# Drehrumbum/viterbi.dll

Measured on AMD Instinct MI355X. Metric: decoded Mbit/s per GPU on batched 768-bit DAB FIC frames; bit-exact vs AVX2 ref, higher is better.
Workload: dtype u8

## Files before the change

### __graft_entry__.py

```python
import os
import sys

ROOT = os.path.dirname(os.path.abspath(__file__))
if ROOT not in sys.path:
    sys.path.insert(0, ROOT)

import _vitpkg


def build():
    V = _vitpkg.load_package()
    V.build(force=False)
    V.lib()
    for sym in V.EXPORTS:
        getattr(V.lib(), sym)
    diag = os.path.join(os.path.dirname(V.LIB_PATH_DEFAULT), "libviterbi_diag.so")
    if not os.path.exists(diag) or os.path.getmtime(diag) < os.path.getmtime(V.LIB_PATH_DEFAULT):
        V.build(extra=["-DVIT_DIAG_SPEC"], out=diag)
    O = _vitpkg.load_oracle()
    O.build()
    O.lib()
    if _vitpkg.load_ref().build():
        _vitpkg.load_ref().lib()


def smoke():
    import numpy as np
    import torch

    V = _vitpkg.load_package()
    O = _vitpkg.load_oracle()
    assert torch.cuda.is_available(), "smoke() needs a GPU"
    assert V.device_count() >= 1, "libviterbi found no gfx950 device"
    assert V.initialize()
    framebits, n = 768, 64
    sym = np.concatenate([O.noisy_frames(n // 2, framebits, seed=7),
                          O.uniform_symbols((n // 2) * O.sym_len(framebits), seed=9).reshape(n // 2, -1)])
    want = O.decode_batch(framebits, sym, ge=True)
    d_sym = torch.from_numpy(sym).to("cuda:0")
    d_out = torch.zeros((n, framebits // 8), dtype=torch.uint8, device="cuda:0")
    V.decode_batch_dev(d_sym, d_out, framebits, n)
    torch.cuda.synchronize()
    got = d_out.cpu().numpy()
    assert np.array_equal(got, want), "GPU decode differs from the oracle"
    reps = 65
    d_big = d_sym.repeat(reps, 1)
    d_big_out = torch.zeros((n * reps, framebits // 8), dtype=torch.uint8, device="cuda:0")
    V.decode_batch_dev(d_big, d_big_out, framebits, n * reps)
    torch.cuda.synchronize()
    assert bool((d_big_out.view(reps, n, -1) == d_out.unsqueeze(0)).all()), "packed kernel differs from the oracle"
    rc, one = V.deconvolve(framebits, sym[0].astype(np.uint32))
    assert rc == 0 and np.array_equal(one, want[0])
    rs = 12
    rng = np.random.default_rng(3)
    cols = np.stack([O.rs_encode(rng.integers(0, 256, 110, dtype=np.uint8)) for _ in range(rs)], axis=1)
    p = cols.reshape(-1).copy()
    p[5 * rs + 3] ^= 0x5A
    p[77 * rs + 3] ^= 0x11
    p[9 * rs + 7] ^= 0xC3
    rc_ref, out_ref = O.rs_check_superframe(p, rs)
    rc_gpu, out_gpu = V.RScheckSuperframe(p, 0, rs)
    assert rc_gpu == rc_ref == 3 and np.array_equal(out_gpu, out_ref)
    print("smoke ok: %d + %d frames bit-exact (latency + packed kernel), deconvolve rc=0, RScheckSuperframe=%d"
          % (n, n * reps, rc_gpu))


if __name__ == "__main__":
    {"build": build, "smoke": smoke}[sys.argv[1] if len(sys.argv) > 1 else "build"]()
```

### viterbi.dll_amd/csrc/vit_pk.hip

```cpp
#include <cstdlib>
#include <mutex>

#include "vit_internal.h"
#include "vit_pk_dev.h"

namespace {

constexpr int TAB_BYTES = 2048;
constexpr int DEC_BLOCK = 512;
constexpr unsigned PK_SPLIT_DEN = 8;

#ifndef VIT_TAB_STATIC
#define VIT_TAB_STATIC 1
#endif
struct Lanes {
    u32 toff[5];
};


#ifndef VIT_SWZ_ALL
#define VIT_SWZ_ALL 1
#endif
#ifndef VIT_K3
#define VIT_K3 2
// ... 90 lines not shown
        return;
#endif
#if VIT_PAIR_LSB
        const u32 z = (u32)__builtin_amdgcn_ds_bpermute((int)((lane & 1u) << 2), (int)W(n0));
#else
        const u32 z = (u32)__builtin_amdgcn_ds_swizzle((int)W(n0), 0);
#endif
        exchange<4 - RHO>(A, B, W(n0), W(n1), lane);
#if VIT_K3 == 2
        u32 K;
        {
            const u32 w = z + C.rc;
            asm("v_pk_ashrrev_i16 %0, 15, %1 op_sel_hi:[0,1]\n\t"
                "v_and_or_b32 %0, %0, %2, %3"
                : "=&v"(K)
                : "v"(w), "s"(0x003F003Fu), "v"(C.hi));
        }
#elif VIT_K3
        u32 K;
        asm("v_pk_add_u16 %0, %1, %2\n\t"
            "v_pk_ashrrev_i16 %0, 15, %0 op_sel_hi:[0,1]\n\t"
            "v_and_or_b32 %0, %0, %3, %4"
            : "=&v"(K)
            : "v"(z), "s"(C.rc + 0x00010000u), "s"(0x003F003Fu), "v"(C.hi));
#else
        const u32 w = z + C.rc;
        const u32 t = (w >> 15) & 0x00010001u;
        const u32 K = t * 63u + C.hi;
#endif
        A = W(__builtin_elementwise_sub_sat(U(A), U(K)));
        B = W(__builtin_elementwise_sub_sat(U(B), U(K)));
    } else {
#ifdef VIT_DIAG_SKIP_X
        if constexpr (RHO == 2) {
            A = W(n0);
            B = W(n1);
            return;
        }
#endif
        exchange<4 - RHO>(A, B, W(n0), W(n1), lane);
    }
}

template <int V, int J, int JEND, bool HIST>
struct Steps {
    static DEV void run(u32& A, u32& B, u32& acc0, u32& acc1, const char* tab, const Lanes& L, u32 lane,
                        const Consts& C) {
        constexpr int RHO = (V + J) % 5;
#if VIT_TAB_STATIC
        const u32 mt = *reinterpret_cast<const __attribute__((address_space(3))) u32*>(L.toff[RHO] + (u32)(J * 64));
#else
        const u32 mt = *reinterpret_cast<const u32*>(tab + L.toff[RHO] + J * 64);
#endif
        acs_step<RHO, J, HIST>(A, B, acc0, acc1, mt, lane, C);
        Steps<V, J + 1, JEND, HIST>::run(A, B, acc0, acc1, tab, L, lane, C);
    }
};
template <int V, int JEND, bool HIST>
struct Steps<V, JEND, JEND, HIST> {
    static DEV void run(u32&, u32&, u32&, u32&, const char*, const Lanes&, u32, const Consts&) {}
};
template <bool HIST, int N = 16>
DEV void steps16(u32 v, u32& A, u32& B, u32& acc0, u32& acc1, const char* th, const Lanes& L, u32 lane, const Consts& C) {
    switch (v) {
        case 0: Steps<0, 0, N, HIST>::run(A, B, acc0, acc1, th, L, lane, C); break;
        case 1: Steps<1, 0, N, HIST>::run(A, B, acc0, acc1, th, L, lane, C); break;
        case 2: Steps<2, 0, N, HIST>::run(A, B, acc0, acc1, th, L, lane, C); break;
        case 3: Steps<3, 0, N, HIST>::run(A, B, acc0, acc1, th, L, lane, C); break;
        default: Steps<4, 0, N, HIST>::run(A, B, acc0, acc1, th, L, lane, C); break;
    }
}
DEV void steps6(u32 v, u32& A, u32& B, u32& acc0, u32& acc1, const char* th, const Lanes& L, u32 lane, const Consts& C) {
    steps16<true, 6>(v, A, B, acc0, acc1, th, L, lane, C);
    acc0 >>= 7;
    acc1 >>= 7;
}

typedef u32 v32u __attribute__((ext_vector_type(32)));
constexpr u32 VREG_BLOCKS = 32;

constexpr u32 DUMP_GROUP = 16;
constexpr u32 SEG_BLOCKS = VREG_BLOCKS + DUMP_GROUP + 1u;

__host__ __device__ inline u32 pk_reg_blocks(u32 nb) {
    if (nb <= DUMP_GROUP + 1u) return 0;
    const u32 r = nb - (DUMP_GROUP + 1u);
    return r < VREG_BLOCKS ? r : VREG_BLOCKS;
}
__host__ __device__ inline u32 pk_img_stride(u32 maxfb) { return ((maxfb + 31u) >> 5) + 2u; }
__host__ __device__ inline u32 pk_scratch_words(u32 maxfb) {
    u32 nblk = (maxfb + VIT_TAIL + 15u) >> 4;
    if (nblk > SEG_BLOCKS) nblk = SEG_BLOCKS;
    const u32 tail = (nblk - pk_reg_blocks(nblk)) * 16u;
    const u32 span = tail > 256u ? tail : 256u;
    const u32 bl = 5u * ((span + 79u) / 80u);
    return (bl + 31u) >> 5;
}
struct PkLayout {
    u32 dec_bytes;
    u32 img_off;
    u32 total;
    u32 maxfb;
};
__host__ __device__ inline PkLayout pk_layout(u32 maxfb) {
    const u32 nb = (maxfb + VIT_TAIL + 15u) >> 4;
    PkLayout l;
    l.maxfb = maxfb;
    l.dec_bytes = (nb - pk_reg_blocks(nb) - 1u) * DEC_BLOCK;
    const u32 scratch = 64u * 4u * pk_scratch_words(maxfb), img = 16u * pk_img_stride(maxfb);
    u32 tabregion = DEC_BLOCK + scratch + img;
    tabregion = tabregion > (u32)TAB_BYTES ? ((tabregion + 15u) & ~15u) : (u32)TAB_BYTES;
    l.img_off = l.dec_bytes + DEC_BLOCK + scratch;
    l.total = l.dec_bytes + tabregion;
    return l;
}

constexpr u32 P_ZERO = 252u;
#ifndef VIT_TB_WARM
#define VIT_TB_WARM 30
#endif
#ifndef VIT_TB16
#define VIT_TB16 (VIT_TB_WARM == 30)
#endif
constexpr u32 TB_WARM = VIT_TB_WARM;
#ifndef VIT_TB_WARM_HARD
#define VIT_TB_WARM_HARD 90
#endif
#ifndef VIT_TB_HARD_MISSES
#define VIT_TB_HARD_MISSES 8
#endif
constexpr u32 TB_WARM_HARD = VIT_TB_WARM_HARD, TB_HARD_MISSES = VIT_TB_HARD_MISSES;

#ifdef VIT_DIAG_SPEC
__device__ unsigned long long g_diag_spec[8];
#define SPEC_COUNT(i) do { if (lane == 0) atomicAdd(&g_diag_spec[i], 1ull); } while (0)
#define SPEC_COUNT_N(i, n) do { if (lane == 0) atomicAdd(&g_diag_spec[i], (unsigned long long)(n)); } while (0)
#else
#define SPEC_COUNT(i) do { } while (0)
#endif

DEV u32 dec_slot(u32 lane) { return acs_pair(lane) * 256u + (31u - acs_l5(lane)) * 8u; }

template <int JJ>
DEV void tb_step(u32& PC, u32& kb, u32 x) {
    const u32 w = *reinterpret_cast<const __attribute__((address_space(3))) unsigned short*>((x & ~511u) | PC);
    kb = __builtin_amdgcn_ubfe(w, (x >> 5) & 15u, 1u);
    const u32 t = ((PC >> (JJ - 2)) & 4u) | (kb << JJ);
    PC = bfi((1u << JJ) | 4u, t, PC);
}

template <bool RECORD, int JA>
DEV void tb_loop(u32& PC, u32* scratch, int i_from, int i_to, bool on, u32 i_start, u32 xbase) {
    u32 cur = 0;
    for (int i = i_from; i >= i_to; i -= 5) {
#define TB_ONE(K)                                                                  \
    {                                                                              \
        const int ii = i - (K);                                                    \
        u32 kb = 0;                                                                \
        if (on && (u32)ii <= i_start) tb_step<3 + (JA + (K)) % 5>(PC, kb, xbase + ((u32)ii << 5)); \
        if (RECORD) {                                                              \
            cur |= kb << (ii & 31);                                                \
            if ((ii & 31) == 0) {                                                  \
                if (on) scratch[ii >> 5] = cur;                                    \
                cur = 0;                                                           \
            }                                                                      \
        }                                                                          \
    }
        TB_ONE(0) TB_ONE(1) TB_ONE(2) TB_ONE(3) TB_ONE(4)
#undef TB_ONE
    }
}
template <bool RECORD>
DEV void tb_run(u32& PC, u32* scratch, int i_from, int i_to, bool on, u32 i_start, u32 xbase, u32 j0) {
    switch ((j0 + 1u) % 5u) {
        case 0: tb_loop<RECORD, 0>(PC, scratch, i_from, i_to, on, i_start, xbase); break;
        case 1: tb_loop<RECORD, 1>(PC, scratch, i_from, i_to, on, i_start, xbase); break;
        case 2: tb_loop<RECORD, 2>(PC, scratch, i_from, i_to, on, i_start, xbase); break;
        case 3: tb_loop<RECORD, 3>(PC, scratch, i_from, i_to, on, i_start, xbase); break;
        default: tb_loop<RECORD, 4>(PC, scratch, i_from, i_to, on, i_start, xbase); break;
    }
}

#ifndef VIT_TB_INLINE
#define VIT_TB_INLINE 1
#endif
#if VIT_TB_INLINE
DEV
#else
__device__ __attribute__((noinline))
#endif
u32 traceback_part(const char* dec, u32* scratch, u32* img, u32 fstride, u32 lane, u32 ts, u32 te, u32 te_max,
                       u32 slot0, u32 P_top, u32& warm, u32 dmask = 0xFFFFFFFFu) {
#ifdef VIT_DIAG_NO_TB
    return P_top;
#endif
    const u32 fi = lane >> 4, q = lane & 15u;
    const u32 span = te_max > ts ? te_max - ts : 0u;
    if (span == 0) return P_top;
    const u32 BL = 5u * ((span + 79u) / 80u);
    const u32 tbase = ts + q * BL;
    const bool has_work = tbase < te;
    const u32 i_last = has_work ? te - 1u - tbase : 0u;
    const u32 q_top = te > ts ? (te - 1u - ts) / BL : 0u;
    const u32 i_warm = BL - 1u + warm;
    const u32 i_start = i_last < i_warm ? i_last : i_warm;
    const bool fixed = has_work && i_last <= i_warm;
    const u32 C = (fi >> 1) * 256u + (fi & 1u) * 2u;
    const u32 dbase = (u32)(uintptr_t)(const __attribute__((address_space(3))) char*)dec;
    if (dbase & 511u) __builtin_trap();
    const u32 xbase = ((tbase - slot0 * 16u) << 5) + dbase;
    const u32 j0 = (4u + 5u - ((ts + 5u - 1u) % 5u)) % 5u;
    const u32 PC_top = P_top | C;

    u32 P = fixed ? PC_top : (P_ZERO | C), P_out = PC_top;
    tb_run<false>(P, scratch, (int)i_warm, (int)BL, has_work, i_start, xbase, j0);
    u32 P_in = P;
    tb_run<true>(P, scratch, (int)BL - 1, 0, has_work, i_start, xbase, j0);
    if (has_work) P_out = P;
    for (int pass = 0; pass < 17; pass++) {
        const u32 nxt = __shfl_down(P_out, 1);
        const u32 new_in = (q < q_top) ? nxt : PC_top;
        const bool changed = has_work && !fixed && new_in != P_in;
        const unsigned long long miss = __ballot(changed);
        if (miss == 0) break;
#ifdef VIT_DIAG_SPEC
        if (pass == 0 && warm == TB_WARM && (u32)__popcll(miss) >= TB_HARD_MISSES) SPEC_COUNT(7);
#endif
        if (pass == 0 && warm == TB_WARM && (u32)__popcll(miss) >= TB_HARD_MISSES) warm = TB_WARM_HARD;
        if (changed) P_in = new_in;
        P = new_in;
        tb_run<true>(P, scratch, (int)BL - 1, 0, changed, BL - 1u, xbase, j0);
        if (changed) P_out = P;
    }
    if (has_work) {
        const u32 nvalid = i_last + 1u < BL ? i_last + 1u : BL;
        const u32 nw = (BL + 31u) >> 5;
        for (u32 w = 0; w < nw; w++) {
            const u32 lo = 32u * w;
            const u32 cnt = nvalid > lo ? nvalid - lo : 0u;
            const u32 mask = cnt >= 32u ? 0xFFFFFFFFu : ((1u << cnt) - 1u);
            const u32 val = ~scratch[w] & mask;
            const u32 b0 = tbase - VIT_TAIL + lo;
            const u32 d = b0 >> 5, sft = b0 & 31u;
            if (val) {
                atomicOr(&img[fi * fstride + (d & dmask)], val << sft);
                if (sft) atomicOr(&img[fi * fstride + ((d + 1u) & dmask)], val >> (32u - sft));
            }
        }
    }
    return __shfl(P_out, (int)(fi * 16u)) & 0xFCu;
}

struct Tb16 {
    u32 sh[5], jj[5], mk[5];
};
DEV u32 bfi_v(u32 mask, u32 a, u32 b) {
    u32 d;
    asm("v_bfi_b32 %0, %1, %2, %3" : "=v"(d) : "v"(mask), "v"(a), "v"(b));
    return d;
}
template <int II, bool REC>
DEV void tb16_step(u32& PC, u32& cur, const Tb16& L) {
    constexpr int r = II % 5, blk = (6 + II) >> 4, idx = (6 + II) & 15;
    const u32 w = *reinterpret_cast<const __attribute__((address_space(3))) unsigned short*>(PC + (u32)(blk * DEC_BLOCK));
    u32 kb;
    asm("v_bfe_u32 %0, %1, %2, 1" : "=v"(kb) : "v"(w), "n"(idx));
    const u32 m = (PC >> L.sh[r]) & 4u;
    const u32 t = (kb << L.jj[r]) | m;
    PC = bfi_v(L.mk[r], t, PC);
    if constexpr (REC) cur |= kb << II;
}
template <int IFROM, int ITO, bool REC>
struct Tb16Run {
    static DEV void run(u32& PC, u32& cur, const Tb16& L) {
        tb16_step<IFROM, REC>(PC, cur, L);
        if constexpr (IFROM > ITO) Tb16Run<IFROM - 1, ITO, REC>::run(PC, cur, L);
    }
};
template <bool SPEC = false, bool TOMEM = false>
DEV u32 traceback_part16(const char* dec, u32* img, u32 fstride, u32 lane, u32 lo, u32 nl, u32 slot0, u32 P_top, u32 dmask,
                         uint8_t* gout = nullptr, u32* p_spec = nullptr, u32* misses = nullptr) {
#ifdef VIT_DIAG_NO_TB
    return P_top;
#endif
    constexpr int W = 30;
    const u32 fi = lane >> 4, q = lane & 15u;
    const u32 tbase = lo + q * 16u;
    const bool has_work = q < nl;
    const u32 above = SPEC ? 3u : nl - q;
    const bool fixed = has_work && above <= 2u;
    const u32 C = (fi >> 1) * 256u + (fi & 1u) * 2u;
    const u32 dbase = (u32)(uintptr_t)(const __attribute__((address_space(3))) char*)dec;
    if (dbase & 511u) __builtin_trap();
    const u32 bbq = dbase + ((lo >> 4) - slot0 + q) * DEC_BLOCK;
    Tb16 L;
    {
        const u32 c = (tbase + 4u) % 5u;
#pragma unroll
        for (int r = 0; r < 5; r++) {
            const u32 e = (c + r) % 5u, JJ = 7u - e;
            L.sh[r] = JJ - 2u;
            L.jj[r] = JJ;
            L.mk[r] = (1u << JJ) | 4u;
        }
    }
    const u32 PC_top = P_top | C;
    u32 P = (fixed ? PC_top : (P_ZERO | C)) | bbq, P_out = PC_top, cur = 0;
    if (has_work && above >= 3u) Tb16Run<15 + W, 32, false>::run(P, cur, L);
    if (has_work && above >= 2u) Tb16Run<31, 16, false>::run(P, cur, L);
    u32 P_in = P & 0x1FFu;
    if (has_work) {
        Tb16Run<15, 0, true>::run(P, cur, L);
        P_out = P & 0x1FFu;
    }
    for (int pass = 0; pass < 17; pass++) {
        const u32 nxt = (u32)__builtin_amdgcn_update_dpp(0, (int)P_out, 0x101, 0xF, 0xF, true);
        const u32 new_in = (q + 1u < nl) ? nxt : (SPEC ? P_in : PC_top);
        const bool changed = has_work && !fixed && new_in != P_in;
        if constexpr (SPEC) {
            const unsigned long long miss = __ballot(changed);
            if (pass == 0) *misses = (u32)__popcll(miss);
            if (miss == 0) break;
        } else {
#ifdef VIT_DIAG_SPEC
            {
                const unsigned long long miss = __ballot(changed);
                if (pass == 0) SPEC_COUNT_N(5, __popcll(miss));
                if (miss) SPEC_COUNT(6);
            }
#endif
            if (!__any(changed)) break;
        }
        if (changed) {
            P_in = new_in;
            P = new_in | bbq;
            cur = 0;
            Tb16Run<15, 0, true>::run(P, cur, L);
            P_out = P & 0x1FFu;
        }
    }
    if (has_work) {
        const u32 h = (tbase - VIT_TAIL) >> 4;
        if constexpr (TOMEM) {
            const u32 v = __builtin_bitreverse32(~cur & 0xFFFFu);
            gout[2u * h] = (uint8_t)(v >> 24);
            gout[2u * h + 1u] = (uint8_t)(v >> 16);
        } else {
            reinterpret_cast<unsigned short*>(img + fi * fstride)[((h >> 1) & dmask) * 2u + (h & 1u)] = (unsigned short)~cur;
        }
    }
    if constexpr (SPEC) *p_spec = __shfl(P_in, (int)(fi * 16u + nl - 1u)) & 0xFCu;
    return __shfl(P_out, (int)(fi * 16u)) & 0xFCu;
}

#ifdef VIT_DIAG_TIMES
__device__ unsigned long long g_diag_times[16384 * 4];
#endif
template <bool SYM32, bool ROT>
__global__ __launch_bounds__(64, 4) void vit_pk_kernel(const uint8_t* __restrict__ sym, uint8_t* __restrict__ out,
                                                        const vit_frame_desc* __restrict__ desc, u32 framebits_uniform,
                                                        long long nframes, PkLayout lay, u32 vmax,
                                                        const unsigned* __restrict__ split_gate, u32 renorm_c) {
    if (split_gate && (unsigned long long)*split_gate * PK_SPLIT_DEN >= (unsigned long long)nframes) return;
#ifdef VIT_DIAG_TIMES
    const unsigned long long diag_t0 = __builtin_amdgcn_s_memrealtime();
#endif
    extern __shared__ __attribute__((aligned(16))) char lds[];
    char* dec = lds;
    char* tab = lds + lay.dec_bytes;
    u32* img = reinterpret_cast<u32*>(lds + lay.img_off);
    const u32 lane = threadIdx.x;
    const long long f0 = (long long)blockIdx.x * 4;
    u32 prio_slot = 0;
#if VIT_PRIO
    {
        u32 hwid;
        asm volatile("s_getreg_b32 %0, hwreg(HW_REG_HW_ID)" : "=s"(hwid));
        prio_slot = hwid & 3u;
#ifdef VIT_PRIO_FIRST
// ... 132 lines not shown
    __syncthreads();
#pragma nounroll
    for (u32 i = lane; i < 4u * fstride; i += 64u) img[i] = 0;

#ifdef VIT_DIAG_TIMES
    const unsigned long long diag_t1 = __builtin_amdgcn_s_memrealtime();
#endif
    const u32 fi = lane >> 4;
    const u32 t_fb = fi == 0 ? fbits[0] : fi == 1 ? fbits[1] : fi == 2 ? fbits[2] : fbits[3];
    const u32 t_T = t_fb ? t_fb + VIT_TAIL : 0u;
    u32* scratch = reinterpret_cast<u32*>(tab + DEC_BLOCK) + lane * pk_scratch_words(maxfb);
#if VIT_TB16
    if (fbits[0] == fbits[1] && fbits[1] == fbits[2] && fbits[2] == fbits[3] && (maxfb & 15u) == 0) {
        u32 hi = T_max, slot0 = R, P16 = P_ZERO;
        for (;;) {
            const u32 lo = hi > 256u + VIT_TAIL ? hi - 256u : VIT_TAIL;
            P16 = traceback_part16(dec, img, fstride, lane, lo, (hi - lo) >> 4, slot0, P16, 0xFFFFFFFFu);
            if (lo == VIT_TAIL) break;
            const u32 d = slot0 < DUMP_GROUP ? slot0 : DUMP_GROUP;
            __syncthreads();
            for (u32 sl = DUMP_GROUP; sl >= d; sl--)
                *reinterpret_cast<uint2*>(dec + sl * DEC_BLOCK + dslot) = *reinterpret_cast<const uint2*>(dec + (sl - d) * DEC_BLOCK + dslot);
            const u32 g0 = slot0 - d;
#pragma unroll
            for (u32 b = 0; b < VREG_BLOCKS; b++)
                if (b >= g0 && b < slot0)
                    *reinterpret_cast<uint2*>(dec + (b - g0) * DEC_BLOCK + dslot) = make_uint2(r1[b], r0[b]);
            __syncthreads();
            slot0 = g0;
            hi = lo;
        }
    } else {
#endif
    const u32 t_lo = R * 16u;
    u32 warm = TB_WARM;
    u32 P_part = traceback_part(dec, scratch, img, fstride, lane, t_lo > VIT_TAIL ? t_lo : VIT_TAIL, t_T, T_max, R,
                                P_ZERO, warm);
    for (u32 g1 = R; g1 > 0;) {
        const u32 g0 = g1 > DUMP_GROUP ? g1 - DUMP_GROUP : 0u;
        __syncthreads();
#pragma unroll
        for (u32 b = 0; b < VREG_BLOCKS; b++)
            if (b >= g0 && b < g1)
                *reinterpret_cast<uint2*>(dec + (b - g0) * DEC_BLOCK + dslot) = make_uint2(r1[b], r0[b]);
        __syncthreads();
        const u32 tsg = g0 ? g0 * 16u : VIT_TAIL, tend = g1 * 16u;
        const u32 te = t_T < tend ? t_T : tend, te_max = T_max < tend ? T_max : tend;
        const u32 P_top = t_T > tend ? P_part : P_ZERO;
        P_part = traceback_part(dec, scratch, img, fstride, lane, tsg, te, te_max, g0, P_top, warm);
        g1 = g0;
    }
#if VIT_TB16
    }
#endif
    __syncthreads();

#ifdef VIT_DIAG_TIMES
    if (threadIdx.x == 0 && blockIdx.x < 16384u) {
        u32 hwid;
        asm volatile("s_getreg_b32 %0, hwreg(HW_REG_HW_ID)" : "=s"(hwid));
        g_diag_times[blockIdx.x * 4u + 0u] = diag_t0;
        g_diag_times[blockIdx.x * 4u + 1u] = diag_t1;
        g_diag_times[blockIdx.x * 4u + 2u] = __builtin_amdgcn_s_memrealtime();
        g_diag_times[blockIdx.x * 4u + 3u] = hwid;
    }
#endif
    {
        const u32 k = lane >> 4, j = lane & 15u;
        const u32 fb_k = k == 0 ? fbits[0] : k == 1 ? fbits[1] : k == 2 ? fbits[2] : fbits[3];
        const size_t oo_k = k == 0 ? ooff[0] : k == 1 ? ooff[1] : k == 2 ? ooff[2] : ooff[3];
        const u32 nbytes = (fb_k + 7u) >> 3;
        uint8_t* o = out + oo_k;
        const u32* im = img + k * fstride;
        if ((((u32)oo_k | nbytes) & 3u) == 0) {
#pragma nounroll
            for (u32 m = j; m < (nbytes >> 2); m += 16u)
                reinterpret_cast<u32*>(o)[m] = __builtin_bswap32(__builtin_bitreverse32(im[m]));
        } else {
#pragma nounroll
            for (u32 b = j; b < nbytes; b += 16u) {
                const u32 byte = (im[b >> 2] >> (8u * (b & 3u))) & 0xFFu;
                o[b] = (uint8_t)(__builtin_bitreverse32(byte) >> 24);
            }
        }
    }
}

constexpr u32 LONG_LDS_BLOCKS = DUMP_GROUP + 1u;
constexpr u32 LONG_KEEP = DUMP_GROUP;
constexpr u32 SPEC_BLOCKS = LONG_LDS_BLOCKS + 2u;

constexpr u32 IMG_RING = 16;

__host__ __device__ inline PkLayout pk_layout_long(u32 maxfb) {
    PkLayout l;
    l.maxfb = maxfb;
    l.dec_bytes = DUMP_GROUP * DEC_BLOCK;
    const u32 scratch = 64u * 4u * pk_scratch_words(maxfb), img = 4u * 4u * IMG_RING;
    u32 tabregion = DEC_BLOCK + scratch + img;
    tabregion = tabregion > (u32)TAB_BYTES ? ((tabregion + 15u) & ~15u) : (u32)TAB_BYTES;
    l.img_off = l.dec_bytes + DEC_BLOCK + scratch;
    l.total = l.dec_bytes + tabregion;
    return l;
}
static_assert(SPEC_BLOCKS * DEC_BLOCK <= DUMP_GROUP * DEC_BLOCK + (u32)TAB_BYTES, "an in-flight part must fit dec + the dead table");

struct Carry {
    u32 a0, b0, a1, b1, a2, b2, a3, b3;
};
DEV void carry_put(Carry& c, int d, u32 x, u32 y) {
    asm volatile(
        "s_cmp_lt_i32 %[d], 16\n\t"
        "s_cbranch_scc1 .Lcy_end%=\n\t"
        "s_cmp_lg_u32 %[d], 16\n\t"
        "s_cbranch_scc1 .Lcy_1%=\n\t"
        "v_mov_b32 %[a0], %[x]\n\t"
        "v_mov_b32 %[b0], %[y]\n\t"
        "s_branch .Lcy_end%=\n"
        ".Lcy_1%=:\n\t"
        "s_cmp_lg_u32 %[d], 17\n\t"
        "s_cbranch_scc1 .Lcy_2%=\n\t"
        "v_mov_b32 %[a1], %[x]\n\t"
        "v_mov_b32 %[b1], %[y]\n\t"
        "s_branch .Lcy_end%=\n"
        ".Lcy_2%=:\n\t"
        "s_cmp_lg_u32 %[d], 18\n\t"
        "s_cbranch_scc1 .Lcy_3%=\n\t"
        "v_mov_b32 %[a2], %[x]\n\t"
        "v_mov_b32 %[b2], %[y]\n\t"
        "s_branch .Lcy_end%=\n"
        ".Lcy_3%=:\n\t"
        "v_mov_b32 %[a3], %[x]\n\t"
        "v_mov_b32 %[b3], %[y]\n"
        ".Lcy_end%=:"
        : [a0] "+v"(c.a0), [b0] "+v"(c.b0), [a1] "+v"(c.a1), [b1] "+v"(c.b1), [a2] "+v"(c.a2), [b2] "+v"(c.b2), [a3] "+v"(c.a3), [b3] "+v"(c.b3)
        : [d] "s"(d), [x] "v"(x), [y] "v"(y)
        : "scc");
}
DEV void carry_to_lds(const Carry& c, char* dec, u32 dslot, u32 first, u32 n) {
    if (n > 0u) *reinterpret_cast<uint2*>(dec + (first + 0u) * DEC_BLOCK + dslot) = make_uint2(c.a0, c.b0);
    if (n > 1u) *reinterpret_cast<uint2*>(dec + (first + 1u) * DEC_BLOCK + dslot) = make_uint2(c.a1, c.b1);
    if (n > 2u) *reinterpret_cast<uint2*>(dec + (first + 2u) * DEC_BLOCK + dslot) = make_uint2(c.a2, c.b2);
    if (n > 3u) *reinterpret_cast<uint2*>(dec + (first + 3u) * DEC_BLOCK + dslot) = make_uint2(c.a3, c.b3);
}
DEV u32 pack_rows(u32 P) {
    return (u32)__builtin_amdgcn_readlane((int)P, 0) | ((u32)__builtin_amdgcn_readlane((int)P, 16) << 8) |
           ((u32)__builtin_amdgcn_readlane((int)P, 32) << 16) | ((u32)__builtin_amdgcn_readlane((int)P, 48) << 24);
}

#ifndef VIT_LONG_BASE_PRIO
#define VIT_LONG_BASE_PRIO 1
#endif
#ifndef VIT_LONG_INFLIGHT
#define VIT_LONG_INFLIGHT 1
#endif

DEV void wave_sync() { asm volatile("s_waitcnt lgkmcnt(0)" ::: "memory"); }

template <bool SYM32>
__global__ __launch_bounds__(64, 4) void vit_pk_long_kernel(const uint8_t* __restrict__ sym, uint8_t* __restrict__ out,
                                                             const vit_frame_desc* __restrict__ desc,
                                                             u32 framebits_uniform, long long nframes, PkLayout lay,
                                                             uint2* spill, u32 spill_blocks, unsigned* counter,
                                                             u32 ngroups, u32 short_max,
                                                             const unsigned* __restrict__ split_gate, u32 renorm_c, u32 nsimd) {
    extern __shared__ __attribute__((aligned(16))) char lds[];
// ... 392 lines not shown
#endif
bool vit_pk_supported(uint32_t max_framebits) {
    if (max_framebits < 2 || max_framebits > PK_MAX_FRAMEBITS || (max_framebits % 2u) != 0) return false;
    const u32 nblk = (max_framebits + VIT_TAIL + 15u) >> 4;
    return (nblk <= SEG_BLOCKS ? pk_layout(max_framebits) : pk_layout_long(max_framebits)).total <= 160u * 1024u;
}

struct ScratchCtx {
    void* buf = nullptr;
    size_t cap = 0;
    hipEvent_t ev = nullptr;
    int dev = -1;
    bool bins_clean = false;
    hipStream_t side = nullptr;
    hipEvent_t ev_fork = nullptr, ev_join = nullptr;
    void drop_side() {
        if (side) (void)hipStreamDestroy(side);
        if (ev_fork) (void)hipEventDestroy(ev_fork);
        if (ev_join) (void)hipEventDestroy(ev_join);
        side = nullptr;
        ev_fork = ev_join = nullptr;
    }
    ~ScratchCtx() {
        drop_side();
        if (buf) (void)hipFree(buf);
        if (ev) (void)hipEventDestroy(ev);
    }
};
constexpr int PK_MAX_DEVS = 64;
struct ScratchCtxs {
    ScratchCtx by_dev[PK_MAX_DEVS];
};
thread_local ScratchCtxs t_scratch;
constexpr size_t SCRATCH_HDR = 16384;
constexpr int64_t SORT_MIN_FRAMES = 16;

bool sort_enabled() {
    static const bool on = getenv("VITERBI_AMD_NO_SORT") == nullptr;
    return on;
}

hipError_t vit_launch_pk(const void* d_symbols, bool sym32, uint8_t* d_out, const vit_frame_desc* d_desc,
                         uint32_t framebits, uint32_t max_framebits, int64_t nframes, hipStream_t stream, bool renorm_ge) {
    const u32 rc = pk_renorm_const(renorm_ge);
    const uint8_t* d_sym = static_cast<const uint8_t*>(d_symbols);
    if (sym32 && (reinterpret_cast<uintptr_t>(d_symbols) & 15u)) return hipErrorInvalidValue;
    if (nframes <= 0) return hipSuccess;
    if (!vit_pk_supported(max_framebits)) return hipErrorInvalidValue;
    hipError_t e;
    int dev = 0;
    if ((e = hipGetDevice(&dev)) != hipSuccess) return e;
    {
        static uint64_t optin_done = 0;
        const void* ks[6] = {reinterpret_cast<const void*>(vit_pk_kernel<false, false>),
                             reinterpret_cast<const void*>(vit_pk_kernel<true, false>),
                             reinterpret_cast<const void*>(vit_pk_kernel<false, true>),
                             reinterpret_cast<const void*>(vit_pk_kernel<true, true>),
                             reinterpret_cast<const void*>(vit_pk_long_kernel<false>),
                             reinterpret_cast<const void*>(vit_pk_long_kernel<true>)};
        if ((e = vit_optin_dynamic_lds(ks, 6, 160 * 1024, dev, &optin_done)) != hipSuccess) return e;
    }
    const long long groups = (nframes + 3) / 4;
    if (groups > 0x7FFFFFFFLL) return hipErrorInvalidValue;
    const u32 nblk = (max_framebits + VIT_TAIL + 15u) >> 4;
#ifdef VIT_FORCE_LONG
    const bool is_long = true;
#else
    const bool is_long = nblk > SEG_BLOCKS;
#endif
    const bool sort = d_desc != nullptr && nframes >= SORT_MIN_FRAMES && sort_enabled();
    const PkLayout lay = is_long ? pk_layout_long(max_framebits) : pk_layout(max_framebits);
    long long grid = groups;
    if (is_long) {
        u32 per_cu = (160u * 1024u) / lay.total;
        if (per_cu > 16u) per_cu = 16u;
        grid = (long long)per_cu * vit_device_cus(dev);
        if (grid > groups) grid = groups;
    }
    const bool need_counter = is_long;
    auto launch_short = [&](long long g, const PkLayout& l, u32 vmax, const unsigned* gate, bool may_rotate) {
        u32 per_cu = (160u * 1024u) / l.total;
        if (per_cu > 16u) per_cu = 16u;
        const bool rot = may_rotate && g <= (long long)per_cu * vit_device_cus(dev) && g > 4ll * vit_device_cus(dev);
#define VIT_LAUNCH_SHORT(S32, R)                                                                                          \
    hipLaunchKernelGGL((vit_pk_kernel<S32, R>), dim3((unsigned)g), dim3(64), l.total, stream, d_sym, d_out, d_desc, framebits, \
                       (long long)nframes, l, vmax, gate, rc)
        if (sym32) {
            if (rot) VIT_LAUNCH_SHORT(true, true);
            else VIT_LAUNCH_SHORT(true, false);
        } else {
            if (rot) VIT_LAUNCH_SHORT(false, true);
            else VIT_LAUNCH_SHORT(false, false);
        }
#undef VIT_LAUNCH_SHORT
    };
    if (!need_counter && !sort) {
        launch_short(grid, lay, lay.maxfb, nullptr, true);
        return hipGetLastError();
    }
    const u32 spill_blocks = is_long ? nblk - LONG_KEEP : 0u;
    const size_t desc_bytes = sort ? (((size_t)nframes * sizeof(vit_frame_desc) + 255u) & ~(size_t)255u) : 0u;
    const size_t need = SCRATCH_HDR + desc_bytes + (size_t)grid * spill_blocks * DEC_BLOCK;
    if (dev < 0 || dev >= PK_MAX_DEVS) return hipErrorInvalidDevice;
    ScratchCtx& sc = t_scratch.by_dev[dev];
    if (sc.cap < need) {
        if (sc.buf) (void)hipFree(sc.buf);
        sc.buf = nullptr;
        sc.cap = 0;
        sc.bins_clean = false;
        if (sc.ev) (void)hipEventDestroy(sc.ev);
        sc.ev = nullptr;
        if ((e = hipMalloc(&sc.buf, need + need / 4)) != hipSuccess) return e;
        sc.cap = need + need / 4;
        sc.dev = dev;
        if ((e = hipEventCreateWithFlags(&sc.ev, hipEventDisableTiming)) != hipSuccess) return e;
    } else if ((e = hipStreamWaitEvent(stream, sc.ev, 0)) != hipSuccess) {
        return e;
    }
    char* base = static_cast<char*>(sc.buf);
    if (sort) {
        vit_frame_desc* sorted = reinterpret_cast<vit_frame_desc*>(base + SCRATCH_HDR);
        if ((e = vit_sort_descs_launch(d_desc, sorted, nframes, max_framebits, reinterpret_cast<unsigned*>(base + 256),
                                       stream, &sc.bins_clean, reinterpret_cast<unsigned*>(base))) != hipSuccess)
            return e;
        d_desc = sorted;
    }
    unsigned* counter = reinterpret_cast<unsigned*>(base);
    if (need_counter && !sort && (e = hipMemsetAsync(base, 0, 256, stream)) != hipSuccess) return e;
    if (is_long) {
        const u32 short_max = sort ? PK_SHORT_MAX : 0u;
        const unsigned* gate = sort ? reinterpret_cast<const unsigned*>(base + 256) + VIT_SORT_BINS + ((PK_SHORT_MAX + 7u) >> 3) : nullptr;
        uint2* spill = reinterpret_cast<uint2*>(base + SCRATCH_HDR + desc_bytes);
        hipStream_t ls = stream;
        if (short_max) {
            if (!sc.side) {
                if ((e = hipStreamCreateWithFlags(&sc.side, hipStreamNonBlocking)) != hipSuccess) return e;
                if ((e = hipEventCreateWithFlags(&sc.ev_fork, hipEventDisableTiming)) != hipSuccess) return e;
                if ((e = hipEventCreateWithFlags(&sc.ev_join, hipEventDisableTiming)) != hipSuccess) return e;
            }
            if ((e = hipEventRecord(sc.ev_fork, stream)) != hipSuccess) return e;
            if ((e = hipStreamWaitEvent(sc.side, sc.ev_fork, 0)) != hipSuccess) return e;
            ls = sc.side;
        }
        if (sym32)
            hipLaunchKernelGGL(vit_pk_long_kernel<true>, dim3((unsigned)grid), dim3(64), lay.total, ls, d_sym, d_out,
                               d_desc, framebits, (long long)nframes, lay, spill, spill_blocks, counter, (u32)groups,
                               short_max, gate, rc, 4u * (u32)vit_device_cus(dev));
        else
            hipLaunchKernelGGL(vit_pk_long_kernel<false>, dim3((unsigned)grid), dim3(64), lay.total, ls, d_sym, d_out,
                               d_desc, framebits, (long long)nframes, lay, spill, spill_blocks, counter, (u32)groups,
                               short_max, gate, rc, 4u * (u32)vit_device_cus(dev));
        if (short_max && (e = hipGetLastError()) == hipSuccess) {
            const PkLayout lsh = pk_layout(PK_SHORT_MAX);
            launch_short(groups, lsh, max_framebits, gate, false);
            if ((e = hipGetLastError()) != hipSuccess) return e;
            if ((e = hipEventRecord(sc.ev_join, sc.side)) != hipSuccess) return e;
            if ((e = hipStreamWaitEvent(stream, sc.ev_join, 0)) != hipSuccess) return e;
        }
    } else {
        launch_short(grid, lay, lay.maxfb, nullptr, true);
    }
    if ((e = hipGetLastError()) != hipSuccess) return e;
    return hipEventRecord(sc.ev, stream);
}
```

Baseline: 120,100.

## Add a compile-time specialised kernel for fixed 768-bit FIC frames

Adds a templated kernel, vit_pk_fixed_kernel<768>, whose block counts, LDS offsets, image stride and loop bounds are all compile-time constants. It uses static shared memory, precomputes the traceback lane geometry once and rotates it at compile time, and fully unrolls the output copy. The launcher dispatches to it when framebits and maxfb are 768 and there is no sort descriptor or gate. The aim is to remove runtime layout arithmetic, branches and per-part geometry recomputation from the hot path, at the cost of more code and a second build variant to maintain.

```diff
diff --git a/__graft_entry__.py b/__graft_entry__.py
--- a/__graft_entry__.py
+++ b/__graft_entry__.py
@@ -17,7 +17,10 @@
     diag = os.path.join(os.path.dirname(V.LIB_PATH_DEFAULT), "libviterbi_diag.so")
     if not os.path.exists(diag) or os.path.getmtime(diag) < os.path.getmtime(V.LIB_PATH_DEFAULT):
         V.build(extra=["-DVIT_DIAG_SPEC"], out=diag)
-    O = _vitpkg.load_oracle()
+    general = os.path.join(os.path.dirname(V.LIB_PATH_DEFAULT), "libviterbi_general.so")
+    if not os.path.exists(general) or os.path.getmtime(general) < os.path.getmtime(V.LIB_PATH_DEFAULT):
+        V.build(extra=["-DVIT_FIC_FIXED=0"], out=general)
+    O =_vitpkg.load_oracle()
     O.build()
     O.lib()
     if _vitpkg.load_ref().build():
diff --git a/viterbi.dll_amd/csrc/vit_pk.hip b/viterbi.dll_amd/csrc/vit_pk.hip
--- a/viterbi.dll_amd/csrc/vit_pk.hip
+++ b/viterbi.dll_amd/csrc/vit_pk.hip
@@ -196,13 +196,13 @@
 constexpr u32 DUMP_GROUP = 16;
 constexpr u32 SEG_BLOCKS = VREG_BLOCKS + DUMP_GROUP + 1u;
 
-__host__ __device__ inline u32 pk_reg_blocks(u32 nb) {
+__host__ __device__ constexpr inline u32 pk_reg_blocks(u32 nb) {
     if (nb <= DUMP_GROUP + 1u) return 0;
     const u32 r = nb - (DUMP_GROUP + 1u);
     return r < VREG_BLOCKS ? r : VREG_BLOCKS;
 }
-__host__ __device__ inline u32 pk_img_stride(u32 maxfb) { return ((maxfb + 31u) >> 5) + 2u; }
-__host__ __device__ inline u32 pk_scratch_words(u32 maxfb) {
+__host__ __device__ constexpr inline u32 pk_img_stride(u32 maxfb) { return ((maxfb + 31u) >> 5) + 2u; }
+__host__ __device__ constexpr inline u32 pk_scratch_words(u32 maxfb) {
     u32 nblk = (maxfb + VIT_TAIL + 15u) >> 4;
     if (nblk > SEG_BLOCKS) nblk = SEG_BLOCKS;
     const u32 tail = (nblk - pk_reg_blocks(nblk)) * 16u;
@@ -216,9 +216,9 @@
     u32 total;
     u32 maxfb;
 };
-__host__ __device__ inline PkLayout pk_layout(u32 maxfb) {
+__host__ __device__ constexpr inline PkLayout pk_layout(u32 maxfb) {
     const u32 nb = (maxfb + VIT_TAIL + 15u) >> 4;
-    PkLayout l;
+    PkLayout l{};
     l.maxfb = maxfb;
     l.dec_bytes = (nb - pk_reg_blocks(nb) - 1u) * DEC_BLOCK;
     const u32 scratch = 64u * 4u * pk_scratch_words(maxfb), img = 16u * pk_img_stride(maxfb);
@@ -368,6 +368,30 @@
 struct Tb16 {
     u32 sh[5], jj[5], mk[5];
 };
+DEV Tb16 tb16_lane(u32 tbase) {
+    Tb16 L;
+    const u32 c = (tbase + 4u) % 5u;
+#pragma unroll
+    for (int r = 0; r < 5; r++) {
+        const u32 e = (c + r) % 5u, JJ = 7u - e;
+        L.sh[r] = JJ - 2u;
+        L.jj[r] = JJ;
+        L.mk[r] = (1u << JJ) | 4u;
+    }
+    return L;
+}
+template <u32 S>
+DEV Tb16 tb16_rotate(const Tb16& a) {
+    Tb16 L;
+#pragma unroll
+    for (int r = 0; r < 5; r++) {
+        const int k = (r + 5 - (int)(S % 5u)) % 5;
+        L.sh[r] = a.sh[k];
+        L.jj[r] = a.jj[k];
+        L.mk[r] = a.mk[k];
+    }
+    return L;
+}
 DEV u32 bfi_v(u32 mask, u32 a, u32 b) {
     u32 d;
     asm("v_bfi_b32 %0, %1, %2, %3" : "=v"(d) : "v"(mask), "v"(a), "v"(b));
@@ -391,9 +415,9 @@
         if constexpr (IFROM > ITO) Tb16Run<IFROM - 1, ITO, REC>::run(PC, cur, L);
     }
 };
-template <bool SPEC = false, bool TOMEM = false>
+template <bool SPEC = false, bool TOMEM = false, bool GEO = false>
 DEV u32 traceback_part16(const char* dec, u32* img, u32 fstride, u32 lane, u32 lo, u32 nl, u32 slot0, u32 P_top, u32 dmask,
-                         uint8_t* gout = nullptr, u32* p_spec = nullptr, u32* misses = nullptr) {
+                         uint8_t* gout = nullptr, u32* p_spec = nullptr, u32* misses = nullptr, const Tb16* geo = nullptr) {
 #ifdef VIT_DIAG_NO_TB
     return P_top;
 #endif
@@ -405,10 +429,14 @@
     const bool fixed = has_work && above <= 2u;
     const u32 C = (fi >> 1) * 256u + (fi & 1u) * 2u;
     const u32 dbase = (u32)(uintptr_t)(const __attribute__((address_space(3))) char*)dec;
-    if (dbase & 511u) __builtin_trap();
+    if constexpr (!GEO) {
+        if (dbase & 511u) __builtin_trap();
+    }
     const u32 bbq = dbase + ((lo >> 4) - slot0 + q) * DEC_BLOCK;
     Tb16 L;
-    {
+    if constexpr (GEO) {
+        L = *geo;
+    } else {
         const u32 c = (tbase + 4u) % 5u;
 #pragma unroll
         for (int r = 0; r < 5; r++) {
@@ -707,6 +735,239 @@
                 const u32 byte = (im[b >> 2] >> (8u * (b & 3u))) & 0xFFu;
                 o[b] = (uint8_t)(__builtin_bitreverse32(byte) >> 24);
             }
+        }
+    }
+}
+
+#ifndef VIT_FIC_FIXED
+#define VIT_FIC_FIXED 1
+#endif
+#ifndef VIT_FIC_FIXED_SPLIT
+#define VIT_FIC_FIXED_SPLIT 1
+#endif
+template <u32 FB>
+struct PkFixed {
+    static constexpr u32 T = FB + VIT_TAIL;
+    static constexpr u32 NB = (T + 15u) >> 4;
+    static constexpr u32 R = pk_reg_blocks(NB);
+    static constexpr u32 LD = NB - R - 1u;
+    static constexpr u32 TAB_OFF = LD * DEC_BLOCK;
+    static constexpr u32 IMG_OFF = TAB_OFF + DEC_BLOCK;
+    static constexpr u32 FSTRIDE = FB / 32u;
+    static constexpr u32 LDS_BYTES = TAB_OFF + (u32)TAB_BYTES;
+    static constexpr u32 SYM_STEPS = T;
+    static constexpr u32 OUT_BYTES = FB / 8u;
+    static_assert(FB % 32u == 0 && FB >= 32u, "whole image dwords, an even number of 16-step blocks below the last one");
+    static_assert(VIT_STEPS6 && (T & 15u) == 6u, "the last block has six steps");
+    static_assert(NB <= SEG_BLOCKS && (R & 1u) == 0 && (LD & 1u) == 0 && R + 3u <= NB, "one segment, cut into pairs of blocks");
+    static_assert(LD <= DUMP_GROUP, "the traceback window is dec + one block");
+    static_assert(IMG_OFF + 16u * FSTRIDE <= LDS_BYTES, "the image fits the dead table region");
+    static_assert(TAB_OFF % 512u == 0, "tb16_step selects the block with the address bits above 511");
+    static_assert(LDS_BYTES == pk_layout(FB).total, "as many waves per CU as the general kernel");
+};
+
+template <class G, u32 HI, u32 SLOT0>
+DEV void fixed_traceback(char* dec, u32* img, u32 lane, u32 dslot, const v32u r0, const v32u r1, u32 P, const Tb16 L) {
+    constexpr u32 LO = HI > 256u + VIT_TAIL ? HI - 256u : VIT_TAIL;
+    static_assert(LO % 16u == VIT_TAIL && (LO >> 4) >= SLOT0 && (HI >> 4) - SLOT0 <= DUMP_GROUP, "the part lies in the window");
+    P = traceback_part16<false, false, true>(dec, img, G::FSTRIDE, lane, LO, (HI - LO) >> 4, SLOT0, P, 0xFFFFFFFFu, nullptr,
+                                             nullptr, nullptr, &L);
+    if constexpr (LO != VIT_TAIL) {
+        constexpr u32 D = SLOT0 < DUMP_GROUP ? SLOT0 : DUMP_GROUP, G0 = SLOT0 - D;
+        static_assert(D >= 1u, "there are blocks below this part");
+        constexpr u32 LO2 = LO > 256u + VIT_TAIL ? LO - 256u : VIT_TAIL;
+        __syncthreads();
+#pragma unroll
+        for (u32 sl = DUMP_GROUP; sl >= D; sl--)
+            *reinterpret_cast<uint2*>(dec + sl * DEC_BLOCK + dslot) = *reinterpret_cast<const uint2*>(dec + (sl - D) * DEC_BLOCK + dslot);
+#pragma unroll
+        for (u32 b = G0; b < SLOT0; b++)
+            *reinterpret_cast<uint2*>(dec + (b - G0) * DEC_BLOCK + dslot) = make_uint2(r1[b], r0[b]);
+        __syncthreads();
+        fixed_traceback<G, LO, G0>(dec, img, lane, dslot, r0, r1, P, tb16_rotate<LO - LO2>(L));
+    }
+}
+
+template <u32 FB, bool SYM32, bool ROT>
+__global__ __launch_bounds__(64, 4) void vit_pk_fixed_kernel(const uint8_t* __restrict__ sym, uint8_t* __restrict__ out,
+                                                              long long nframes, u32 renorm_c) {
+    typedef PkFixed<FB> G;
+#ifdef VIT_DIAG_TIMES
+    const unsigned long long diag_t0 = __builtin_amdgcn_s_memrealtime();
+#endif
+    __shared__ __attribute__((aligned(512))) char lds[G::LDS_BYTES];
+    char* dec = lds;
+    char* tab = lds + G::TAB_OFF;
+    u32* img = reinterpret_cast<u32*>(lds + G::IMG_OFF);
+    const u32 lane = threadIdx.x;
+    u32 prio_slot = 0;
+#if VIT_PRIO
+    {
+        u32 hwid;
+        asm volatile("s_getreg_b32 %0, hwreg(HW_REG_HW_ID)" : "=s"(hwid));
+        prio_slot = hwid & 3u;
+        switch (VIT_PRIO_MAP(hwid & 3u)) {
+            case 0: __builtin_amdgcn_s_setprio(0); break;
+            case 1: __builtin_amdgcn_s_setprio(1); break;
+            case 2: __builtin_amdgcn_s_setprio(2); break;
+            default: __builtin_amdgcn_s_setprio(3); break;
+        }
+    }
+#endif
+    constexpr u32 SB = SYM32 ? 4u : 1u, STEP_BYTES = 4u * SB, FRAME_BYTES = G::SYM_STEPS * STEP_BYTES;
+    const long long f0 = (long long)blockIdx.x * 4;
+    const long long left = nframes - f0;
+    const u32 nvalid = left >= 4 ? 4u : (u32)left;
+    const uint8_t* gsym = sym + (size_t)f0 * FRAME_BYTES;
+    uint8_t* gout = out + (size_t)f0 * G::OUT_BYTES;
+
+    const u32 l5 = acs_l5(lane);
+    const u32 dslot = dec_slot(lane);
+    Lanes L;
+    load_toff(L, lane);
+#if VIT_TAB_STATIC
+    Lanes L1;
+    {
+        const u32 tb = (u32)(uintptr_t)(const __attribute__((address_space(3))) char*)tab;
+#pragma unroll
+        for (int rho = 0; rho < 5; rho++) {
+            L.toff[rho] += tb;
+            L1.toff[rho] = L.toff[rho] + 1024u;
+            asm volatile("" : "+v"(L1.toff[rho]));
+        }
+    }
+#endif
+    Consts C;
+    C.hi = HI;
+    C.rc = renorm_c;
+    asm volatile("" : "+v"(C.hi));
+    const u32 tau = lane >> 1, pp = lane & 1u;
+    u32 ka = 2u * pp, kb = 2u * pp + 1u;
+    if (nvalid < 4u) {
+        ka = ka < nvalid ? ka : 0u;
+        kb = kb < nvalid ? kb : 0u;
+    }
+    const u32 a_off = ka * FRAME_BYTES + tau * STEP_BYTES, b_off = kb * FRAME_BYTES + tau * STEP_BYTES;
+    typedef typename RawStep<SYM32>::type Raw;
+    auto load32 = [&](u32 off, u32 rb) {
+        return *reinterpret_cast<const Raw*>(gsym + (size_t)rb * (16u * STEP_BYTES) + off);
+    };
+    u32 sel[4];
+    {
+        const u32 hb = (tau & 1u) ? 0x0C000C00u : 0x0D000D00u;
+#pragma unroll
+        for (int k = 0; k < 4; k++) sel[k] = hb | (0x00040000u + 0x00010001u * k);
+    }
+    const PrepassLane PL = prepass_lane(lane);
+    u32 A = l5 == 0 ? 0u : 0x003F003Fu, B = 0x003F003Fu;
+    u32 acc0 = 0, acc1 = 0;
+    v32u r0, r1;
+
+    {
+        Raw sa = load32(a_off, 0u), sb = load32(b_off, 0u);
+        u32 v = 0;
+        auto rotate = [&](const u32 rbx) {
+            if constexpr (ROT) {
+                switch ((prio_slot + rbx) & 3u) {
+                    case 0: __builtin_amdgcn_s_setprio(0); break;
+                    case 1: __builtin_amdgcn_s_setprio(1); break;
+                    case 2: __builtin_amdgcn_s_setprio(2); break;
+                    default: __builtin_amdgcn_s_setprio(3); break;
+                }
+            }
+        };
+        auto put_reg = [&](const u32 rbx) {
+            u32 i = rbx;
+            asm volatile("" : "+s"(i));
+            r0[i] = acc0;
+            r1[i] = acc1;
+        };
+        auto put_lds = [&](const u32 rbx) {
+            u32 rbs = rbx;
+            asm volatile("" : "+s"(rbs));
+            *reinterpret_cast<uint2*>(dec + (rbs - G::R) * DEC_BLOCK + dslot) = make_uint2(acc1, acc0);
+        };
+        auto trip = [&](const u32 rb, auto&& put) {
+            u32 rbs = rb;
+            asm volatile("" : "+s"(rbs));
+            rotate(rb);
+            __syncthreads();
+            prepass(pack_step(sa), pack_step(sb), tab, PL, sel);
+            sa = load32(a_off, rbs + 2u);
+            sb = load32(b_off, rbs + 2u);
+            __syncthreads();
+            steps16<true>(v, A, B, acc0, acc1, tab, L, lane, C);
+            put(rb);
+            v = v == 4 ? 0 : v + 1;
+            rotate(rb + 1u);
+            steps16<true>(v, A, B, acc0, acc1, tab, L1, lane, C);
+            put(rb + 1u);
+            v = v == 4 ? 0 : v + 1;
+        };
+#if VIT_FIC_FIXED_SPLIT
+        for (u32 rb = 0; rb < G::R; rb += 2u) trip(rb, put_reg);
+        for (u32 rb = G::R; rb + 3u < G::NB; rb += 2u) trip(rb, put_lds);
+#else
+        for (u32 rb = 0; rb + 3u < G::NB; rb += 2u)
+            trip(rb, [&](const u32 rbx) {
+                if (rbx < G::R) put_reg(rbx);
+                else put_lds(rbx);
+            });
+#endif
+        {
+            constexpr u32 rb = G::NB - 3u;
+            rotate(rb);
+            __syncthreads();
+            prepass(pack_step(sa), pack_step(sb), tab, PL, sel);
+            sa = sb = Raw{};
+            if (tau < G::T - (rb + 2u) * 16u) {
+                sa = load32(a_off, rb + 2u);
+                sb = load32(b_off, rb + 2u);
+            }
+            __syncthreads();
+            Steps<rb % 5u, 0, 16, true>::run(A, B, acc0, acc1, tab, L, lane, C);
+            put_lds(rb);
+            rotate(rb + 1u);
+            Steps<(rb + 1u) % 5u, 0, 16, true>::run(A, B, acc0, acc1, tab, L1, lane, C);
+            put_lds(rb + 1u);
+        }
+        {
+            constexpr u32 rb = G::NB - 1u;
+            rotate(rb);
+            __syncthreads();
+            prepass(pack_step(sa), pack_step(sb), tab, PL, sel);
+            __syncthreads();
+            Steps<rb % 5u, 0, 6, true>::run(A, B, acc0, acc1, tab, L, lane, C);
+            acc0 >>= 7;
+            acc1 >>= 7;
+            __syncthreads();
+            put_lds(rb);
+        }
+    }
+    __syncthreads();
+#ifdef VIT_DIAG_TIMES
+    const unsigned long long diag_t1 = __builtin_amdgcn_s_memrealtime();
+#endif
+    fixed_traceback<G, G::T, G::R>(dec, img, lane, dslot, r0, r1, P_ZERO, tb16_lane((G::T > 256u + VIT_TAIL ? G::T - 256u : VIT_TAIL) + (lane & 15u) * 16u));
+    __syncthreads();
+#ifdef VIT_DIAG_TIMES
+    if (threadIdx.x == 0 && blockIdx.x < 16384u) {
+        u32 hwid;
+        asm volatile("s_getreg_b32 %0, hwreg(HW_REG_HW_ID)" : "=s"(hwid));
+        g_diag_times[blockIdx.x * 4u + 0u] = diag_t0;
+        g_diag_times[blockIdx.x * 4u + 1u] = diag_t1;
+        g_diag_times[blockIdx.x * 4u + 2u] = __builtin_amdgcn_s_memrealtime();
+        g_diag_times[blockIdx.x * 4u + 3u] = hwid;
+    }
+#endif
+    {
+        const u32 k = lane >> 4, j = lane & 15u;
+        if (k < nvalid) {
+            u32* o = reinterpret_cast<u32*>(gout + k * G::OUT_BYTES);
+            const u32* im = img + k * G::FSTRIDE;
+#pragma unroll
+            for (u32 m0 = 0; m0 < G::FSTRIDE; m0 += 16u)
+                if (m0 + 16u <= G::FSTRIDE || j < G::FSTRIDE - m0) o[m0 + j] = __builtin_bswap32(__builtin_bitreverse32(im[m0 + j]));
         }
     }
 }
@@ -1265,6 +1526,22 @@
         u32 per_cu = (160u * 1024u) / l.total;
         if (per_cu > 16u) per_cu = 16u;
         const bool rot = may_rotate && g <= (long long)per_cu * vit_device_cus(dev) && g > 4ll * vit_device_cus(dev);
+#if VIT_FIC_FIXED
+        if (!d_desc && !gate && framebits == 768u && l.maxfb == 768u) {
+#define VIT_LAUNCH_FIXED(S32, R)                                                                                          \
+    hipLaunchKernelGGL((vit_pk_fixed_kernel<768u, S32, R>), dim3((unsigned)g), dim3(64), 0, stream, d_sym, d_out, \
+                       (long long)nframes, rc)
+            if (sym32) {
+                if (rot) VIT_LAUNCH_FIXED(true, true);
+                else VIT_LAUNCH_FIXED(true, false);
+            } else {
+                if (rot) VIT_LAUNCH_FIXED(false, true);
+                else VIT_LAUNCH_FIXED(false, false);
+            }
+#undef VIT_LAUNCH_FIXED
+            return;
+        }
+#endif
 #define VIT_LAUNCH_SHORT(S32, R)                                                                                          \
     hipLaunchKernelGGL((vit_pk_kernel<S32, R>), dim3((unsigned)g), dim3(64), l.total, stream, d_sym, d_out, d_desc, framebits, \
                        (long long)nframes, l, vmax, gate, rc)
```

After: 121,800, median of 6. 1.5% higher.
